# 583phoenix-hue/Airfoil-CFD-Tool

Measured on AMD Instinct MI355X. Metric: MLUPS on 4096² fp32 D2Q9 at 1/2/4/8 MI355X; achieved % HBM3E peak, higher is better.
Workload: dtype f32

## Files before the change

### airfoil-cfd-tool_amd/csrc/step_march3.hpp

```cpp
#pragma once
#include "step_march.hpp"

namespace wt {

static constexpr int M3_SREC = 80;
static constexpr int M3_SHALF = 40;
static constexpr int M3_HL = 32;
static constexpr int HL_COLS = 60;
static constexpr int H3_COLS = HL_COLS, H4_COLS = HL_COLS;


__global__ __launch_bounds__(256) void k_seam_flags3(const uint8_t *__restrict__ mask, const uint8_t *__restrict__ bcode, uint8_t *__restrict__ flags3,
                                                     Geom g, int nwin, int win)
{
    const long total = (long)(nwin - 1) * g.nxl;
    const long t = (long)blockIdx.x * 256 + threadIdx.x;
    if (t >= total) return;
    const int x = (int)(t % g.nxl);
    const int b = 1 + (int)(t / g.nxl);
    const uint8_t *m = mask + g.pitch;
    const int gi = x + g.gi0;
    unsigned f = 0;
    for (int r4 = 0; r4 < 4; r4++) {
        const int j = win * b - 2 + r4;
        if (j <= 0 || j >= g.ny - 1 || gi <= 0 || gi >= g.nx_g - 1) continue;
        const long c = (long)x * g.pitch + j;
        if (m[c] == 0 && bcode[c] == 0) f |= 1u << r4;
    }
    flags3[t] = (uint8_t)f;
}
__global__ __launch_bounds__(256) void k_seam_flags4(const uint8_t *__restrict__ mask, const uint8_t *__restrict__ bcode, uint8_t *__restrict__ flags4,
                                                     Geom g, int nwin, int win)
{
    const long total = (long)(nwin - 1) * g.nxl;
    const long t = (long)blockIdx.x * 256 + threadIdx.x;
    if (t >= total) return;
    const int x = (int)(t % g.nxl);
    const int b = 1 + (int)(t / g.nxl);
    const uint8_t *m = mask + g.pitch;
    const int gi = x + g.gi0;
    unsigned f = 0;
    for (int r6 = 0; r6 < 6; r6++) {
        const int j = win * b - 3 + r6;
        if (j <= 0 || j >= g.ny - 1 || gi <= 0 || gi >= g.nx_g - 1) continue;
        const long c = (long)x * g.pitch + j;
        if (m[c] == 0 && bcode[c] == 0) f |= 1u << r6;
    }
    flags4[t] = (uint8_t)f;
}

template <typename T, int FD, typename GET>
__device__ __forceinline__ void halo_step(unsigned sc, const Geom &g, int x, int j, bool plain, GET get, const FastDiv &fdv, T tau, T U0,
                                          T (&o)[9])
{
    if (j >= g.ny || x < 0 || x >= g.nxl) {
#pragma unroll
        for (int k = 0; k < 9; k++) o[k] = T(0);
        return;
    }
    const int gi = x + g.gi0;
    if (plain) {
        T fin[9], rho, ux, uy;
#pragma unroll
        for (int k = 0; k < 9; k++) fin[k] = get(k, -ex_of(k), -ey_of(k));
        collide_t<T, FD>(fin, fdv, tau, o, rho, ux, uy);
    } else if (sc & 256u) {
#pragma unroll
        for (int k = 0; k < 9; k++) o[k] = get(opp_of(k), 0, 0);
    } else if (gi == g.nx_g - 1) {
#pragma unroll
        for (int k = 0; k < 9; k++) o[k] = get(k, -1, 0);
    } else if (gi == 0 || j == g.ny - 1 || j == 0) {
        feq_all<T>(T(1), U0, T(0), o);
    } else {
        T fin[9], rho, ux, uy;
        fin[0] = get(0, 0, 0);
#pragma unroll
        for (int k = 1; k < 9; k++) fin[k] = ((sc >> (k - 1)) & 1u) ? get(opp_of(k), 0, 0) : get(k, -ex_of(k), -ey_of(k));
        collide_t<T, FD>(fin, fdv, tau, o, rho, ux, uy);
    }
}

#ifdef WT_UNIT_CLOCKS
__device__ unsigned long long g_halo_clk[8];
#define H4_STAMP(i) do { const unsigned long long t_ = __builtin_amdgcn_s_memtime(); hst_[i] = t_ - tprev_; tprev_ = t_; } while (0)
#else
#define H4_STAMP(i) do { } while (0)
#endif

template <typename T, int FD>
__device__ __forceinline__ void site_step1_seams(const T *__restrict__ rec, const T (&a)[9], int q0, unsigned sc, const Geom &g, int x, int j,
                                                 const FastDiv &fdv, T tau, T U0, T (&out)[9])
{
    const int gi = x + g.gi0;
    const int e0 = (q0 >> 2) * M3_SHALF + (q0 & 3);
    if (sc & 256u) {
#pragma unroll
        for (int k = 0; k < 9; k++) out[k] = rec[e0 + 4 * opp_of(k)];
    } else if (gi == g.nx_g - 1) {
#pragma unroll
        for (int k = 0; k < 9; k++) out[k] = rec[-M3_SREC + e0 + 4 * k];
    } else if (gi == 0 || j == g.ny - 1 || j == 0) {
        feq_all<T>(T(1), U0, T(0), out);
    } else {
        T fin[9], rho, ux, uy;
        fin[0] = a[0];
#pragma unroll
        for (int k = 1; k < 9; k++) fin[k] = ((sc >> (k - 1)) & 1u) ? rec[e0 + 4 * opp_of(k)] : a[k];
        collide_t<T, FD>(fin, fdv, tau, out, rho, ux, uy);
    }
}

template <typename T, int S, int FD, int DEPTH>
__device__ __forceinline__ void halo_lines_body(const T *__restrict__ fs, const T *__restrict__ seams3, const uint8_t *__restrict__ mask,
                                                const uint8_t *__restrict__ bcode, const uint8_t *__restrict__ flags, T *__restrict__ hl, const Geom &g, int nwin, int use_seams,
                                                const FastDiv &fdv, T tau, T U0, int xb0, int nbx)
{
    constexpr int WIN = 64 * S, NL = DEPTH - 1;
    constexpr int C1 = HL_COLS + 2 * NL, R1 = 2 * NL;
    constexpr int C2 = HL_COLS + 2 * (NL - 1), R2 = 2 * (NL - 1);
    constexpr int PADK = sizeof(T) == 4 ? 10 : 9;
    __shared__ __attribute__((aligned(32))) T l1[C1][R1][PADK];
    __shared__ T l2[DEPTH == 4 ? C2 : 1][DEPTH == 4 ? R2 : 1][9];
    __shared__ __attribute__((aligned(32))) T lv0[HL_COLS][2][4];
    static_assert(sizeof(T) * C1 * R1 * PADK >= sizeof(T) * HL_COLS * M3_HL, "the lines fit into l1");
    T (*ol)[M3_HL] = reinterpret_cast<T (*)[M3_HL]>(&l1[0][0][0]);
    const int b = 1 + (int)(blockIdx.x / nbx);
    const int x0 = (xb0 + (int)(blockIdx.x % nbx)) * HL_COLS;
    const uint8_t *m = mask + g.pitch;
    const T *s = fs + g.pitch;
    typedef T t4 __attribute__((ext_vector_type(4)));
#ifdef WT_UNIT_CLOCKS
    unsigned long long hst_[7] = {0, 0, 0, 0, 0, 0, 0}, tprev_ = __builtin_amdgcn_s_memtime();
#endif
    unsigned fl2 = 0, fl3 = 0, sc2 = 0, sc3 = 0;
    auto site_code = [&](int x, int j) -> unsigned {
        const long c = (long)x * g.pitch + j;
        return (unsigned)bcode[c] | (m[c] ? 256u : 0u);
    };
    if constexpr (DEPTH == 4) {
        const int x = x0 - (NL - 1) + (int)threadIdx.x / R2, j = WIN * b - (NL - 1) + (int)threadIdx.x % R2;
        if (x >= 0 && x < g.nxl) {
            fl2 = flags[(long)(b - 1) * g.nxl + x];
            if (j < g.ny && !((fl2 >> ((int)threadIdx.x % R2 + 1)) & 1)) sc2 = site_code(x, j);
        }
    }
    if (threadIdx.x < 2 * (HL_COLS + 2)) {
        const int x = x0 - 1 + (int)(threadIdx.x >> 1), j = WIN * b - 1 + (int)(threadIdx.x & 1);
        if (x >= 0 && x < g.nxl) {
            fl3 = flags[(long)(b - 1) * g.nxl + x];
            if (j < g.ny && !((fl3 >> (NL - 1 + (int)(threadIdx.x & 1))) & 1)) sc3 = site_code(x, j);
        }
    }
    for (int w = threadIdx.x; w < C1 * R1; w += 256) {
        const int cl = w / R1, r = w % R1;
        const int x = x0 - NL + cl;
        const int j = WIN * b - NL + r;
        T o[9];
#pragma unroll
        for (int k = 0; k < 9; k++) o[k] = T(0);
        if (x >= 0 && x < g.nxl && j < g.ny) {
            T a[9];
            const T *rec = seams3 + ((long)b * (g.nxl + 2) + x + 1) * M3_SREC;
#pragma unroll
            for (int k = 0; k < 9; k++) {
                const int q = 4 - NL + r - ey_of(k);
                a[k] = rec[-(long)ex_of(k) * M3_SREC + (q >> 2) * M3_SHALF + 4 * k + (q & 3)];
            }
            const bool plain = use_seams && ((flags[(long)(b - 1) * g.nxl + x] >> r) & 1) != 0;
            const int o0 = cl - NL;
            if ((r == NL || r == NL - 1) && o0 >= 0 && o0 < HL_COLS) {
                const bool below = r == NL;
                T v0 = below ? a[2] : a[4], v1 = below ? a[5] : a[7], v2 = below ? a[6] : a[8];
                if (!use_seams) {
                    const long c = (long)x * g.pitch + j;
                    if (below) { v0 = s[2 * g.plane + c - 1]; v1 = s[5 * g.plane + c - g.pitch - 1]; v2 = s[6 * g.plane + c + g.pitch - 1]; }
                    else { v0 = s[4 * g.plane + c + 1]; v1 = s[7 * g.plane + c + g.pitch + 1]; v2 = s[8 * g.plane + c - g.pitch + 1]; }
                }
                *reinterpret_cast<t4 *>(&lv0[o0][below ? 0 : 1][0]) = t4{v0, v1, v2, T(0)};
            }
            if (plain) {
                T rho, ux, uy;
                collide_t<T, FD>(a, fdv, tau, o, rho, ux, uy);
            } else if (use_seams) {
                site_step1_seams<T, FD>(rec, a, 4 - NL + r, site_code(x, j), g, x, j, fdv, tau, U0, o);
            } else {
                site_step1<T, FD>(s, m, g, x, j, fdv, tau, U0, o);
            }
        } else {
            const int o0 = cl - NL;
            if ((r == NL || r == NL - 1) && o0 >= 0 && o0 < HL_COLS) *reinterpret_cast<t4 *>(&lv0[o0][r == NL ? 0 : 1][0]) = t4{T(0), T(0), T(0), T(0)};
        }
#pragma unroll
        for (int k = 0; k < 9; k++) l1[cl][r][k] = o[k];
    }
    H4_STAMP(0);
    __syncthreads();
    H4_STAMP(1);
    if constexpr (DEPTH == 4) {
        static_assert(DEPTH != 4 || C2 * R2 == 256, "one level-2 item per thread");
        for (int w = threadIdx.x; w < C2 * R2; w += 256) {
            const int c2 = w / R2, r = w % R2;
            const int x = x0 - (NL - 1) + c2;
            const int j = WIN * b - (NL - 1) + r;
            const bool plain = ((fl2 >> (r + 1)) & 1) != 0;
            auto get = [&](int k, int dx, int dy) { return l1[c2 + 1 + dx][r + 1 + dy][k]; };
            T o[9];
            halo_step<T, FD>(sc2, g, x, j, plain, get, fdv, tau, U0, o);
#pragma unroll
            for (int k = 0; k < 9; k++) l2[c2][r][k] = o[k];
        }
        H4_STAMP(2);
        __syncthreads();
        H4_STAMP(3);
    }
    T wl[3] = {T(0), T(0), T(0)};
    t4 wq[3];
    const bool last_thr = threadIdx.x < 2 * (HL_COLS + 2), asm_thr = threadIdx.x >= 128 && threadIdx.x < 128 + 2 * HL_COLS;
    if (last_thr) {
        const int c = threadIdx.x >> 1, side = threadIdx.x & 1;
        const int x = x0 - 1 + c;
        const int j = WIN * b - 1 + side;
        const bool plain = ((fl3 >> (NL - 1 + side)) & 1) != 0;
        T o[9];
        if constexpr (DEPTH == 4) {
            auto get = [&](int k, int dx, int dy) { return l2[c + 1 + dx][1 + side + dy][k]; };
            halo_step<T, FD>(sc3, g, x, j, plain, get, fdv, tau, U0, o);
        } else {
            auto get = [&](int k, int dx, int dy) { return l1[c + 1 + dx][1 + side + dy][k]; };
            halo_step<T, FD>(sc3, g, x, j, plain, get, fdv, tau, U0, o);
        }
        wl[0] = side ? o[4] : o[2]; wl[1] = side ? o[8] : o[5]; wl[2] = side ? o[7] : o[6];
    } else if (asm_thr) {
        const int t = threadIdx.x - 128, o = t >> 1, side = t & 1;
        auto words = [&](const auto &lk, int c, int r) {
            return side == 0 ? t4{lk[c][r][2], lk[c - 1][r][5], lk[c + 1][r][6], T(0)} : t4{lk[c][r][4], lk[c + 1][r][7], lk[c - 1][r][8], T(0)};
        };
        wq[0] = words(l1, o + NL, NL - 1 + side);
        if constexpr (DEPTH == 4) wq[1] = words(l2, o + NL - 1, NL - 2 + side);
        wq[2] = *reinterpret_cast<const t4 *>(&lv0[o][side][0]);
    }
    H4_STAMP(4);
    __syncthreads();
    if (last_thr) {
        const int c = threadIdx.x >> 1, side = threadIdx.x & 1;
        const int base = 16 * side + 4 * (NL - 1);
        if (c >= 1 && c <= HL_COLS) { ol[c - 1][base] = wl[0]; ol[c - 1][base + 3] = T(0); }
        if (c < HL_COLS) ol[c][base + (side ? 2 : 1)] = wl[1];
        if (c >= 2) ol[c - 2][base + (side ? 1 : 2)] = wl[2];
    } else if (asm_thr) {
        const int t = threadIdx.x - 128, o = t >> 1, side = t & 1;
        *reinterpret_cast<t4 *>(&ol[o][16 * side]) = wq[0];
        if constexpr (DEPTH == 4) *reinterpret_cast<t4 *>(&ol[o][16 * side + 4]) = wq[1];
        *reinterpret_cast<t4 *>(&ol[o][16 * side + 12]) = wq[2];
    }
    __syncthreads();
    {
        const int nlines = g.nxl - x0 < HL_COLS ? g.nxl - x0 : HL_COLS;
        t4 *dst = reinterpret_cast<t4 *>(hl + ((long)b * (g.nxl + 2) + x0 + 1) * M3_HL);
        const t4 *src = reinterpret_cast<const t4 *>(&ol[0][0]);
        for (int t = threadIdx.x; t < nlines * (M3_HL / 4); t += 256) dst[t] = src[t];
    }
    H4_STAMP(5);
#ifdef WT_UNIT_CLOCKS
    if (threadIdx.x == 0) {
        for (int i = 0; i < 7; i++) atomicAdd(&g_halo_clk[i], hst_[i]);
        atomicAdd(&g_halo_clk[7], 1ULL);
    }
#endif
}

template <typename T, int S, int FD>
__global__ __launch_bounds__(256) void k_halo3(const T *__restrict__ fs, const T *__restrict__ seams3, const uint8_t *__restrict__ mask,
                                               const uint8_t *__restrict__ bcode, const uint8_t *__restrict__ flags3, T *__restrict__ hl, Geom g, int nwin, int use_seams,
                                               FastDiv fdv, T tau, T U0, int xb0, int nbx)
{
    halo_lines_body<T, S, FD, 3>(fs, seams3, mask, bcode, flags3, hl, g, nwin, use_seams, fdv, tau, U0, xb0, nbx);
}
template <typename T, int S, int FD>
__global__ __launch_bounds__(256) void k_halo4(const T *__restrict__ fs, const T *__restrict__ seams3, const uint8_t *__restrict__ mask,
                                               const uint8_t *__restrict__ bcode, const uint8_t *__restrict__ flags4, T *__restrict__ hl, Geom g, int nwin, int use_seams,
                                               FastDiv fdv, T tau, T U0, int xb0, int nbx)
{
    halo_lines_body<T, S, FD, 4>(fs, seams3, mask, bcode, flags4, hl, g, nwin, use_seams, fdv, tau, U0, xb0, nbx);
}


#ifdef WT_M3_STAMPS
__device__ unsigned long long g_m3_stamps[8];
#define M3_STAMP(i) do { const unsigned long long t_ = __builtin_amdgcn_s_memtime(); st_[i] += t_ - tprev_; tprev_ = t_; } while (0)
#else
#define M3_STAMP(i) do { } while (0)
#endif

template <typename T, int S>
struct March3Addr {
    MarchAddr<T, S> a;
    __amdgpu_buffer_rsrc_t rs3;
    unsigned voff_lo, voff_hi;
    T *lds_w;
    const char *lds_r;
};

template <bool BODY, bool WANT_MACRO, int FD, int LB, typename T, int S>
__device__ __forceinline__ void march_stage(const MarchParams<T> &p, int c, int j0, int lane, bool far_win, bool nf, bool allsolid,
                                            const T (&feq0)[9], const MV<T, S> (&m158)[3], const MV<T, S> (&Gc)[9], const MV<T, S> (&Gn)[9], T hv,
                                            MV<T, S> (&out)[9], MV<T, S> (&mac)[3], const uint32_t *pre = nullptr)
{
    typedef MV<T, S> V3;
    const Geom &g = p.g;
    constexpr bool OVL = (FD & MARCH_FD_OVL) != 0;
    V3 fin[9];
    fin[0] = Gc[0]; fin[1] = m158[0]; fin[3] = Gn[3];
    fin[2] = m_below_x<LB, OVL>(Gc[2], hv); fin[5] = m_below_x<LB + 1, OVL>(m158[1], hv); fin[6] = m_below_x<LB + 2, OVL>(Gn[6], hv);
    fin[4] = m_above_x<LB, OVL>(Gc[4], hv); fin[8] = m_above_x<LB + 2, OVL>(m158[2], hv); fin[7] = m_above_x<LB + 1, OVL>(Gn[7], hv);
    if (BODY) {
        const int gi = c + g.gi0;
        if (__builtin_expect(gi <= 0 || nf, 0)) {
            auto ownc = [&](int k) { return Gc[k]; };
            uint32_t solid4 = 0, code4 = 0;
            if (nf) {
                if (pre) { solid4 = pre[0]; code4 = pre[1]; }
                else {
                    solid4 = load_site_bytes<S>(p.mask + (long)(c + 1) * g.pitch + site_row<S, OVL>(j0, g.ny));
                    code4 = load_site_bytes<S>(p.bcode + (long)c * g.pitch + site_row<S, OVL>(j0, g.ny));
                }
            }
            const bool any_solid = __ballot(solid4 != 0) != 0ULL;
            if (gi <= 0) {
#pragma unroll
                for (int k = 0; k < 9; k++) out[k] = mv_splat<T, S>(feq0[k]);
                if (WANT_MACRO) { mac[0] = mv_splat<T, S>(T(1)); mac[1] = mv_splat<T, S>(p.U0); mac[2] = mv_splat<T, S>(T(0)); }
            } else if (allsolid) {
#pragma unroll
                for (int k = 0; k < 9; k++) out[k] = Gc[k];
                if (WANT_MACRO) { mac[0] = mv_splat<T, S>(T(1)); mac[1] = mv_splat<T, S>(T(0)); mac[2] = mv_splat<T, S>(T(0)); }
            } else {
                march_bounce<T, S>(fin, code4, ownc);
                march_collide_general<T, S, FD, WANT_MACRO>(fin, solid4, j0, g.ny, p.fdv, p.tau, p.U0, feq0, out, mac);
            }
            if (any_solid && (gi <= 0 || allsolid)) march_solid<T, S, WANT_MACRO>(out, mac, solid4, ownc);
            return;
        }
    }
    march_collide<T, S, FD, WANT_MACRO>(fin, p.fdv, p.tau, out, mac);
    if (far_win) march_far_rows<T, S, WANT_MACRO>(j0, g.ny, p.U0, feq0, out, mac);
}

template <bool EMIT, bool OVL = false, typename T, int S>
__device__ __forceinline__ void march3_store(const March3Addr<T, S> &m, unsigned voff_st, int col, const MV<T, S> (&out)[9], const MV<T, S> (&mac)[3])
{
    const MarchAddr<T, S> &a = m.a;
#pragma unroll
    for (int k = 0; k < 9; k++) bstore<T, S>(a.rd, voff_st, lat_off(a, k, col, 0), out[k]);
    if (EMIT) {
        const unsigned mo = (unsigned)col * a.pitch4;
#pragma unroll
        for (int q = 0; q < 3; q++) bstore<T, S>(a.rm, voff_st, (unsigned)q * a.mp4 + mo, mac[q]);
    }
    if constexpr (!OVL) {
#pragma unroll
        for (int k = 0; k < 9; k++) {
            u2v x;
            __builtin_memcpy(&x, &out[k], 8);
            *reinterpret_cast<u2v *>(m.lds_w + 4 * k) = x;
        }
    }
}
template <typename T, int S>
__device__ __forceinline__ void wait_for_column(const MV<T, S> (&c)[9], T h1)
{
#ifdef WT_M3_NOWAIT
    return;
#endif
    u2v r[9];
#pragma unroll
    for (int k = 0; k < 9; k++) __builtin_memcpy(&r[k], &c[k], 8);
    asm volatile("" ::"v"(r[0]), "v"(r[1]), "v"(r[2]), "v"(r[3]), "v"(r[4]), "v"(r[5]), "v"(r[6]), "v"(r[7]), "v"(r[8]), "v"(h1));
}
template <typename T, int S>
__device__ __forceinline__ void wait_for_column(const MV<T, S> (&c)[9], T h1, T h2)
{
    wait_for_column(c, h1);
#ifndef WT_M3_NOWAIT
    asm volatile("" ::"v"(h2));
#endif
}
template <typename T, int S>
__device__ __forceinline__ void wait_for_column(const MV<T, S> (&c)[9], T h1, T h2, T h3)
{
    wait_for_column(c, h1);
#ifndef WT_M3_NOWAIT
    asm volatile("" ::"v"(h2), "v"(h3));
#endif
}
__device__ __forceinline__ void wait_for_bytes(const SiteBytes &b)
{
#ifndef WT_M3_NOWAIT
    asm volatile("" ::"v"(b.v[0]), "v"(b.v[1]));
#endif
}
template <typename T, int S>
__device__ __forceinline__ void pin_after(const MV<T, S> (&c)[9])
{
    u2v r[9];
#pragma unroll
    for (int k = 0; k < 9; k++) __builtin_memcpy(&r[k], &c[k], 8);
    asm volatile("" ::"v"(r[0]), "v"(r[1]), "v"(r[2]), "v"(r[3]), "v"(r[4]), "v"(r[5]), "v"(r[6]), "v"(r[7]), "v"(r[8]));
}
struct Seam3 { u4v below, above; };
template <bool OVL = false, typename T, int S>
__device__ __forceinline__ Seam3 seam3_fetch(const March3Addr<T, S> &m)
{
    Seam3 r;
    if constexpr (OVL) { r.below = u4v{0, 0, 0, 0}; r.above = r.below; return r; }
    r.below = *reinterpret_cast<const u4v *>(m.lds_r);
    r.above = *reinterpret_cast<const u4v *>(m.lds_r + M3_SHALF * sizeof(T));
    return r;
}
template <bool OVL = false, typename T, int S>
__device__ __forceinline__ void seam3_flush(const March3Addr<T, S> &m, int col, const Seam3 &r)
{
    if constexpr (OVL) return;
    const unsigned so = (unsigned)(col + 1) * (unsigned)(M3_SREC * sizeof(T));
    const u4v d0 = r.below, d1 = r.above;
    __builtin_amdgcn_raw_buffer_store_b128(d0, m.rs3, m.voff_hi, so, 0);
    __builtin_amdgcn_raw_buffer_store_b128(d1, m.rs3, m.voff_lo, so, 0);
    store_data_fence2(d0, d1);
}

template <bool BODY, bool EMIT, int FD, typename T, int S>
__device__ __forceinline__ void march_unit3(const MarchParams<T> &p, March3Addr<T, S> &m, __amdgpu_buffer_rsrc_t rh, unsigned hoff,
                                            int ia, int ib, int uflags, int j0, int lane, bool far_win, ClassMask nonfast_m,
                                            ClassMask solid_m, const T (&feq0)[9])
{
    constexpr bool OVLF = (FD & MARCH_FD_OVL) != 0;
    typedef MV<T, S> V3;
    constexpr unsigned HREC = M3_HL * sizeof(T);
    const Geom &g = p.g;
    const MarchAddr<T, S> &a = m.a;
#define NONFAST(x) (BODY && cm_bit(nonfast_m, (x) - ia + 2))
#define ALLSOLID(x) (BODY && cm_bit(solid_m, (x) - ia + 2))
#define OWN_BUF(x) (a.own_lds + ((x) & 1) * OWN_LDS_BYTES)
#define OWN_NOW(x) do { if (BODY && NONFAST(x)) own_prefetch<T, S, OVLF>(a, (x), OWN_BUF(x)); } while (0)
#define STEP1(x, in, G) march_step1<BODY, FD, T, S, BODY>(p, a, (x), j0, far_win, NONFAST(x), ALLSOLID(x), feq0, in, G, nullptr, OWN_BUF(x))
#define STEP1P(x, in, G, sb) march_step1<BODY, FD, T, S, BODY>(p, a, (x), j0, far_win, NONFAST(x), ALLSOLID(x), feq0, in, G, BODY ? (sb).v : nullptr, OWN_BUF(x))
    const bool outlet = BODY && (uflags & MU_OUTLET_AFTER) != 0;
    const int xend = outlet ? ib : ib + 1;
    V3 s1m[3], s1c[9];
    V3 s2m[3], s2c[9];
    V3 in[9], G1[9], G2[9], mac[3];
#pragma unroll
    for (int k = 0; k < 9; k++) { s1c[k] = mv_splat<T, S>(feq0[k]); s2c[k] = s1c[k]; }
    s1m[0] = s1c[1]; s1m[1] = s1c[5]; s1m[2] = s1c[8];
    s2m[0] = s1c[1]; s2m[1] = s1c[5]; s2m[2] = s1c[8];
    T hv2 = halo_load_x<OVLF, T>(rh, hoff, (unsigned)(ia - 2 > 0 ? ia - 2 : 0) * HREC);
    T hv1 = halo_load_x<OVLF, T>(rh, hoff, (unsigned)(ia - 1 > 0 ? ia - 1 : 0) * HREC);
    T hv0 = halo_load_x<OVLF, T>(rh, hoff, (unsigned)ia * HREC);
    if (!BODY || ia - 2 + g.gi0 >= 0) {
        OWN_NOW(ia - 2);
        march_load_aligned(a, ia - 2, in);
        march_align_in<OVLF>(in, lane, hv2);
        STEP1(ia - 2, in, s1c);
    }
    s1m[0] = s1c[1]; s1m[1] = s1c[5]; s1m[2] = s1c[8];
    if (!BODY || ia - 1 + g.gi0 >= 0) {
        OWN_NOW(ia - 1);
        march_load_aligned(a, ia - 1, in);
        march_align_in<OVLF>(in, lane, hv1);
        STEP1(ia - 1, in, s1c);
    }
    OWN_NOW(ia);
    march_load_aligned(a, ia, in);
    SiteBytes sb0{{0, 0}}, sb1{{0, 0}}, sb2{{0, 0}};
    if (BODY) { sb0 = site_bytes_load<T, S, OVLF>(p, ia, j0); sb1 = site_bytes_load<T, S, OVLF>(p, ia - 1, j0); sb2 = site_bytes_load<T, S, OVLF>(p, ia - 2, j0); wait_for_bytes(sb0); wait_for_bytes(sb1); wait_for_bytes(sb2); }
    wait_for_column(in, hv0, hv1, hv2);
    int seam_col = -1;
#ifdef WT_M3_STAMPS
    unsigned long long st_[8] = {0, 0, 0, 0, 0, 0, 0, 0}, tprev_ = __builtin_amdgcn_s_memtime();
#endif
#pragma unroll 1
    for (int x = ia; x <= xend; x++) {
        V3 nxt[9];
        if (BODY && x + 1 <= xend && NONFAST(x + 1)) own_prefetch<T, S, OVLF>(a, x + 1, OWN_BUF(x + 1));
        march_load_aligned(a, (x + 1 <= xend) ? x + 1 : x, nxt);
        const bool has2 = x - 2 >= ia;
        const int c1 = x - 1, c2 = x - 2;
        const T hvn = halo_load_x<OVLF, T>(rh, hoff, (unsigned)(x + 1) * HREC);
        SiteBytes sbn{{0, 0}};
        if (BODY) sbn = site_bytes_load<T, S, OVLF>(p, x + 1, j0);
        const Seam3 sp = seam3_fetch<OVLF>(m);
        M3_STAMP(0);
        march_align_in<OVLF>(in, lane, hv0);
        STEP1P(x, in, G1, sb0);
        M3_STAMP(1);
        march_stage<BODY, false, FD, 0>(p, c1, j0, lane, far_win, NONFAST(c1), ALLSOLID(c1), feq0, s1m, s1c, G1, hv1, G2, mac, BODY ? sb1.v : nullptr);
#ifdef WT_M3_STAMPS
        pin_after(G2);
#endif
        M3_STAMP(2);
        V3 out[9];
        march_stage<BODY, EMIT, FD, 4>(p, c2, j0, lane, far_win, NONFAST(c2), ALLSOLID(c2), feq0, s2m, s2c, G2, hv2, out, mac, BODY ? sb2.v : nullptr);
        pin_after(out);
        M3_STAMP(3);
        wait_for_column(nxt, hvn);
        if (BODY) { wait_for_bytes(sbn); sb2 = sb1; sb1 = sb0; sb0 = sbn; }
#ifdef WT_M3_STAMPS
        asm volatile("s_waitcnt vmcnt(0)" ::: "memory");
#endif
        M3_STAMP(4);
        hv2 = hv1; hv1 = hv0; hv0 = hvn;
        march3_store<EMIT, OVLF>(m, has2 ? a.voff_st : p.lat_bytes, has2 ? c2 : 0, out, mac);
        seam3_flush<OVLF>(m, seam_col, sp);
        M3_STAMP(5);
        seam_col = has2 ? c2 : seam_col;
        if (BODY && outlet && x == xend) break;
        s2m[0] = s2c[1]; s2m[1] = s2c[5]; s2m[2] = s2c[8];
        s1m[0] = s1c[1]; s1m[1] = s1c[5]; s1m[2] = s1c[8];
#pragma unroll
        for (int k = 0; k < 9; k++) { s2c[k] = G2[k]; s1c[k] = G1[k]; in[k] = nxt[k]; }
    }
#ifdef WT_M3_STAMPS
    if (!BODY && lane == 0) {
        for (int i = 0; i < 6; i++) atomicAdd(&g_m3_stamps[i], st_[i]);
        atomicAdd(&g_m3_stamps[6], (unsigned long long)(xend - ia + 1));
        atomicAdd(&g_m3_stamps[7], 1ULL);
    }
#endif
    if (BODY && outlet) {
        const int co = ib;
        uint32_t solid4 = 0;
        if (NONFAST(co)) solid4 = load_site_bytes<S>(p.mask + (long)(co + 1) * g.pitch + site_row<S, OVLF>(j0, g.ny));
        const bool any_solid = __ballot(solid4 != 0) != 0ULL;
        V3 L2o[9], out[9];
#pragma unroll
        for (int k = 0; k < 9; k++) L2o[k] = s1c[k];
        if (any_solid) { auto own1 = [&](int k) { return G1[k]; }; march_solid<T, S, false>(L2o, mac, solid4, own1); }
        V3 t2m[3];
        t2m[0] = s2c[1]; t2m[1] = s2c[5]; t2m[2] = s2c[8];
        const T hv2t = halo_load_x<OVLF, T>(rh, hoff, (unsigned)(co - 1) * HREC);
        Seam3 sp = seam3_fetch<OVLF>(m);
        march_stage<BODY, EMIT, FD, 4>(p, co - 1, j0, lane, far_win, NONFAST(co - 1), ALLSOLID(co - 1), feq0, t2m, G2, L2o, hv2t, out, mac);
        march3_store<EMIT, OVLF>(m, a.voff_st, co - 1, out, mac);
        seam3_flush<OVLF>(m, seam_col, sp);
        seam_col = co - 1;
#pragma unroll
        for (int k = 0; k < 9; k++) out[k] = G2[k];
        if (EMIT) march_outlet_macro(G2, mac);
        if (any_solid) { auto own2 = [&](int k) { return L2o[k]; }; march_solid<T, S, EMIT>(out, mac, solid4, own2); }
        sp = seam3_fetch<OVLF>(m);
        march3_store<EMIT, OVLF>(m, a.voff_st, co, out, mac);
        seam3_flush<OVLF>(m, seam_col, sp);
        seam_col = co;
    }
    seam3_flush<OVLF>(m, seam_col, seam3_fetch<OVLF>(m));
#undef NONFAST
#undef ALLSOLID
#undef STEP1
#undef STEP1P
#undef OWN_BUF
#undef OWN_NOW
}

template <bool BODY, bool EMIT, int FD, typename T, int S>
__device__ __forceinline__ void march_unit4(const MarchParams<T> &p, March3Addr<T, S> &m, __amdgpu_buffer_rsrc_t rh,
                                            unsigned hoff, int ia, int ib, int uflags, int j0, int lane, bool far_win,
                                            ClassMask nonfast_m, ClassMask solid_m, const T (&feq0)[9])
{
    constexpr bool OVLF = (FD & MARCH_FD_OVL) != 0;
    typedef MV<T, S> V3;
    constexpr unsigned HREC = M3_HL * sizeof(T);
    const Geom &g = p.g;
    const MarchAddr<T, S> &a = m.a;
#define NONFAST(x) (BODY && (x) >= ia - 3 && cm_bit(nonfast_m, (x) - ia + 3))
#define ALLSOLID(x) (BODY && (x) >= ia - 3 && cm_bit(solid_m, (x) - ia + 3))
#define OWN_BUF(x) (a.own_lds + ((x) & 1) * OWN_LDS_BYTES)
#define OWN_NOW(x) do { if (BODY && NONFAST(x)) own_prefetch<T, S, OVLF>(a, (x), OWN_BUF(x)); } while (0)
#define STEP1(x, in, G) march_step1<BODY, FD, T, S, BODY>(p, a, (x), j0, far_win, NONFAST(x), ALLSOLID(x), feq0, in, G, nullptr, OWN_BUF(x))
#define HCOL(c) ((unsigned)((c) > 0 ? (c) : 0) * HREC)
    const bool outlet = BODY && (uflags & MU_OUTLET_AFTER) != 0;
    const int xend = outlet ? ib : ib + 2;
    V3 s1m[3], s1c[9];
    V3 s2m[3], s2c[9];
    V3 s3m[3], s3c[9];
    V3 in[9], G1[9], G2[9], G3[9], mac[3];
#pragma unroll
    for (int k = 0; k < 9; k++) { s1c[k] = mv_splat<T, S>(feq0[k]); s2c[k] = s1c[k]; s3c[k] = s1c[k]; }
    s1m[0] = s1c[1]; s1m[1] = s1c[5]; s1m[2] = s1c[8];
    s2m[0] = s1c[1]; s2m[1] = s1c[5]; s2m[2] = s1c[8];
    s3m[0] = s1c[1]; s3m[1] = s1c[5]; s3m[2] = s1c[8];
    const int xs = ia - 1;
#define LCOL(x) ((BODY && (x) + g.gi0 < 0) ? -g.gi0 : (x))
    T hv3 = halo_load_x<OVLF, T>(rh, hoff, HCOL(xs - 3)), hv2 = halo_load_x<OVLF, T>(rh, hoff, HCOL(xs - 2)), hv1 = halo_load_x<OVLF, T>(rh, hoff, HCOL(xs - 1)),
      hv0 = halo_load_x<OVLF, T>(rh, hoff, HCOL(xs));
    if (!BODY || ia - 3 + g.gi0 >= 0) {
        OWN_NOW(ia - 3);
        march_load_aligned(a, ia - 3, in);
        march_align_in<OVLF>(in, lane, hv2);
        STEP1(ia - 3, in, s1c);
    }
    s1m[0] = s1c[1]; s1m[1] = s1c[5]; s1m[2] = s1c[8];
    if (!BODY || ia - 2 + g.gi0 >= 0) {
        OWN_NOW(ia - 2);
        march_load_aligned(a, ia - 2, in);
        march_align_in<OVLF>(in, lane, hv1);
        STEP1(ia - 2, in, s1c);
    }
    OWN_NOW(xs);
    march_load_aligned(a, LCOL(xs), in);
    SiteBytes sb0{{0, 0}}, sb1{{0, 0}}, sb2{{0, 0}}, sb3{{0, 0}};
    if (BODY) {
        sb0 = site_bytes_load<T, S, OVLF>(p, xs, j0); sb1 = site_bytes_load<T, S, OVLF>(p, xs - 1, j0); sb2 = site_bytes_load<T, S, OVLF>(p, xs - 2, j0); sb3 = site_bytes_load<T, S, OVLF>(p, xs - 3, j0);
        wait_for_bytes(sb0); wait_for_bytes(sb1); wait_for_bytes(sb2); wait_for_bytes(sb3);
    }
    wait_for_column(in, hv0, hv1, hv2);
    wait_for_column(in, hv3);
    int seam_col = -1;
#pragma unroll 1
    for (int x = xs; x <= xend; x++) {
        V3 nxt[9];
        if (BODY && x + 1 <= xend && NONFAST(x + 1)) own_prefetch<T, S, OVLF>(a, x + 1, OWN_BUF(x + 1));
        march_load_aligned(a, (x + 1 <= xend) ? x + 1 : x, nxt);
        const bool has3 = x - 3 >= ia;
        const int c1 = x - 1, c2 = x - 2, c3 = x - 3;
        const T hvn = halo_load_x<OVLF, T>(rh, hoff, HCOL(x + 1));
        SiteBytes sbn{{0, 0}};
        if (BODY) sbn = site_bytes_load<T, S, OVLF>(p, x + 1, j0);
        const Seam3 sp = seam3_fetch<OVLF>(m);
        march_align_in<OVLF>(in, lane, hv0);
        march_step1<BODY, FD, T, S, BODY>(p, a, x, j0, far_win, NONFAST(x), ALLSOLID(x), feq0, in, G1, BODY ? sb0.v : nullptr, OWN_BUF(x));

        march_stage<BODY, false, FD, 0>(p, c1, j0, lane, far_win, NONFAST(c1), ALLSOLID(c1), feq0, s1m, s1c, G1, hv1, G2, mac, BODY ? sb1.v : nullptr);
        march_stage<BODY, false, FD, 4>(p, c2, j0, lane, far_win, NONFAST(c2), ALLSOLID(c2), feq0, s2m, s2c, G2, hv2, G3, mac, BODY ? sb2.v : nullptr);
        V3 out[9];
        march_stage<BODY, EMIT, FD, 8>(p, c3, j0, lane, far_win, NONFAST(c3), ALLSOLID(c3), feq0, s3m, s3c, G3, hv3, out, mac, BODY ? sb3.v : nullptr);
        pin_after(out);
        wait_for_column(nxt, hvn);
        if (BODY) { wait_for_bytes(sbn); sb3 = sb2; sb2 = sb1; sb1 = sb0; sb0 = sbn; }
        hv3 = hv2; hv2 = hv1; hv1 = hv0; hv0 = hvn;
        march3_store<EMIT, OVLF>(m, has3 ? a.voff_st : p.lat_bytes, has3 ? c3 : 0, out, mac);
        seam3_flush<OVLF>(m, seam_col, sp);
        seam_col = has3 ? c3 : seam_col;
        if (BODY && outlet && x == xend) break;
        s3m[0] = s3c[1]; s3m[1] = s3c[5]; s3m[2] = s3c[8];
        s2m[0] = s2c[1]; s2m[1] = s2c[5]; s2m[2] = s2c[8];
        s1m[0] = s1c[1]; s1m[1] = s1c[5]; s1m[2] = s1c[8];
#pragma unroll
        for (int k = 0; k < 9; k++) { s3c[k] = G3[k]; s2c[k] = G2[k]; s1c[k] = G1[k]; in[k] = nxt[k]; }
    }
    if (BODY && outlet) {
        const int co = ib;
        uint32_t solid4 = 0;
        if (NONFAST(co)) solid4 = load_site_bytes<S>(p.mask + (long)(co + 1) * g.pitch + site_row<S, OVLF>(j0, g.ny));
        const bool any_solid = __ballot(solid4 != 0) != 0ULL;
        V3 O2[9], O3[9], L3a[9], out[9], tm[3];
#pragma unroll
        for (int k = 0; k < 9; k++) O2[k] = s1c[k];
        if (any_solid) { auto own = [&](int k) { return G1[k]; }; march_solid<T, S, false>(O2, mac, solid4, own); }
        tm[0] = s2c[1]; tm[1] = s2c[5]; tm[2] = s2c[8];
        march_stage<BODY, false, FD, 4>(p, co - 1, j0, lane, far_win, NONFAST(co - 1), ALLSOLID(co - 1), feq0, tm, G2, O2, halo_load_x<OVLF, T>(rh, hoff, HCOL(co - 1)), L3a, mac);
#pragma unroll
        for (int k = 0; k < 9; k++) O3[k] = G2[k];
        if (any_solid) { auto own = [&](int k) { return O2[k]; }; march_solid<T, S, false>(O3, mac, solid4, own); }
        tm[0] = s3c[1]; tm[1] = s3c[5]; tm[2] = s3c[8];
        Seam3 sp = seam3_fetch<OVLF>(m);
        const bool own2 = co - 2 >= ia;
        march_stage<BODY, EMIT, FD, 8>(p, co - 2, j0, lane, far_win, NONFAST(co - 2), ALLSOLID(co - 2), feq0, tm, G3, L3a, halo_load_x<OVLF, T>(rh, hoff, HCOL(co - 2)), out, mac);
        march3_store<EMIT, OVLF>(m, own2 ? a.voff_st : p.lat_bytes, own2 ? co - 2 : 0, out, mac);
        seam3_flush<OVLF>(m, seam_col, sp);
        seam_col = own2 ? co - 2 : seam_col;
        tm[0] = G3[1]; tm[1] = G3[5]; tm[2] = G3[8];
        sp = seam3_fetch<OVLF>(m);
        march_stage<BODY, EMIT, FD, 8>(p, co - 1, j0, lane, far_win, NONFAST(co - 1), ALLSOLID(co - 1), feq0, tm, L3a, O3, halo_load_x<OVLF, T>(rh, hoff, HCOL(co - 1)), out, mac);
        march3_store<EMIT, OVLF>(m, a.voff_st, co - 1, out, mac);
        seam3_flush<OVLF>(m, seam_col, sp);
        seam_col = co - 1;
#pragma unroll
        for (int k = 0; k < 9; k++) out[k] = L3a[k];
        if (EMIT) march_outlet_macro(L3a, mac);
        if (any_solid) { auto own = [&](int k) { return O3[k]; }; march_solid<T, S, EMIT>(out, mac, solid4, own); }
        sp = seam3_fetch<OVLF>(m);
        march3_store<EMIT, OVLF>(m, a.voff_st, co, out, mac);
        seam3_flush<OVLF>(m, seam_col, sp);
        seam_col = co;
    }
    seam3_flush<OVLF>(m, seam_col, seam3_fetch<OVLF>(m));
#undef NONFAST
#undef ALLSOLID
#undef STEP1
#undef OWN_BUF
#undef OWN_NOW
#undef HCOL
#undef LCOL
}

template <bool BODY, bool EMIT, int FD, typename T, int S>
__device__ __forceinline__ void march_unit3_d2(const MarchParams<T> &p, March3Addr<T, S> &m, __amdgpu_buffer_rsrc_t rh, unsigned hoff, int ia, int ib,
                                               int uflags, int j0, int lane, bool far_win, ClassMask nonfast_m, ClassMask solid_m,
                                               const T (&feq0)[9])
{
    constexpr bool OVLF = (FD & MARCH_FD_OVL) != 0;
    typedef MV<T, S> V3;
    constexpr unsigned HREC = M3_HL * sizeof(T);
    const Geom &g = p.g;
    const MarchAddr<T, S> &a = m.a;
#define NONFAST(x) (BODY && cm_bit(nonfast_m, (x) - ia + 2))
#define ALLSOLID(x) (BODY && cm_bit(solid_m, (x) - ia + 2))
#define STEP1(x, in, G) march_step1<BODY, FD, T, S>(p, a, (x), j0, far_win, NONFAST(x), ALLSOLID(x), feq0, in, G)
    const bool outlet = BODY && (uflags & MU_OUTLET_AFTER) != 0;
    const int xend = ib;
    V3 s1m[3], s1c[9];
    V3 in[9], G1[9], mac[3];
#pragma unroll
    for (int k = 0; k < 9; k++) s1c[k] = mv_splat<T, S>(feq0[k]);
    s1m[0] = s1c[1]; s1m[1] = s1c[5]; s1m[2] = s1c[8];
    T hv1 = halo_load_x<OVLF, T>(rh, hoff, (unsigned)(ia - 1 > 0 ? ia - 1 : 0) * HREC), hv0 = halo_load_x<OVLF, T>(rh, hoff, (unsigned)ia * HREC);
    if (!BODY || ia - 1 + g.gi0 >= 0) {
        march_load_aligned(a, ia - 1, in);
        march_align_in<OVLF>(in, lane, hv1);
        STEP1(ia - 1, in, s1c);
    }
    march_load_aligned(a, ia, in);
    wait_for_column(in, hv0, hv1);
    int seam_col = -1;
#pragma unroll 1
    for (int x = ia; x <= xend; x++) {
        V3 nxt[9];
        march_load_aligned(a, (x + 1 <= xend) ? x + 1 : x, nxt);
        const bool has1 = x - 1 >= ia;
        const int c1 = x - 1;
        const T hvn = halo_load_x<OVLF, T>(rh, hoff, (unsigned)(x + 1) * HREC);
        const Seam3 sp = seam3_fetch<OVLF>(m);
        march_align_in<OVLF>(in, lane, hv0);
        STEP1(x, in, G1);
        V3 out[9];
        march_stage<BODY, EMIT, FD, 0>(p, c1, j0, lane, far_win, NONFAST(c1), ALLSOLID(c1), feq0, s1m, s1c, G1, hv1, out, mac);
        pin_after(out);
        wait_for_column(nxt, hvn);
        hv1 = hv0; hv0 = hvn;
        march3_store<EMIT, OVLF>(m, has1 ? a.voff_st : p.lat_bytes, has1 ? c1 : 0, out, mac);
        seam3_flush<OVLF>(m, seam_col, sp);
        seam_col = has1 ? c1 : seam_col;
        if (BODY && outlet && x == xend) break;
        s1m[0] = s1c[1]; s1m[1] = s1c[5]; s1m[2] = s1c[8];
#pragma unroll
        for (int k = 0; k < 9; k++) { s1c[k] = G1[k]; in[k] = nxt[k]; }
    }
    if (BODY && outlet) {
        const int co = ib;
        uint32_t solid4 = 0;
        if (NONFAST(co)) solid4 = load_site_bytes<S>(p.mask + (long)(co + 1) * g.pitch + site_row<S, OVLF>(j0, g.ny));
        V3 out[9];
#pragma unroll
        for (int k = 0; k < 9; k++) out[k] = s1c[k];
        if (EMIT) march_outlet_macro(s1c, mac);
        if (__ballot(solid4 != 0) != 0ULL) { auto own1 = [&](int k) { return G1[k]; }; march_solid<T, S, EMIT>(out, mac, solid4, own1); }
        const Seam3 sp = seam3_fetch<OVLF>(m);
        march3_store<EMIT, OVLF>(m, a.voff_st, co, out, mac);
        seam3_flush<OVLF>(m, seam_col, sp);
        seam_col = co;
    }
    seam3_flush<OVLF>(m, seam_col, seam3_fetch<OVLF>(m));
#undef NONFAST
#undef ALLSOLID
#undef STEP1
}

static inline MarchRange march_range3(const Geom &g, int depth = 3)
{
    MarchRange r;
    r.i_begin = (g.gi0 == 0) ? 0 : depth - 1;
    r.outlet_after = (g.gi0 + g.nxl == g.nx_g) ? 1 : 0;
    r.i_end = r.outlet_after ? g.nxl - 1 : g.nxl - (depth - 1);
    return r;
}

}
```

Before: 225,500.

## Rewrite fp32 halo-line kernel to process site pairs per thread with packed collide

Adds a new fp32 halo-lines body in which each thread handles two vertically adjacent sites, uses packed f2v loads from LDS and a paired collide routine, and stages intermediate levels in padded LDS with odd-bank column strides. Plain fluid pairs take a fast path with no per-site boundary classification, and assembly of the output lines is split between two thread groups. The aim is to cut per-site overhead and LDS bank conflicts in the halo kernel. The cost is more complex code and more registers per thread. The fp64 path still uses the old body.

```diff
diff --git a/airfoil-cfd-tool_amd/csrc/step_march3.hpp b/airfoil-cfd-tool_amd/csrc/step_march3.hpp
--- a/airfoil-cfd-tool_amd/csrc/step_march3.hpp
+++ b/airfoil-cfd-tool_amd/csrc/step_march3.hpp
@@ -270,19 +270,309 @@
 #endif
 }
 
+struct HaloSite {
+    unsigned rev;
+    bool outlet;
+    bool far;
+    bool zero;
+    bool keep;
+};
+__device__ __forceinline__ HaloSite halo_site(unsigned sc, const Geom &g, int x, int j)
+{
+    HaloSite h;
+    const int gi = x + g.gi0;
+    h.zero = j >= g.ny || x < 0 || x >= g.nxl;
+    const bool solid = (sc & 256u) != 0;
+    h.outlet = !solid && gi == g.nx_g - 1;
+    h.far = !h.zero && !solid && !h.outlet && (gi == 0 || j == g.ny - 1 || j == 0);
+    h.rev = solid ? 0x1ffu : ((h.outlet || h.far) ? 0u : (sc & 0xffu) << 1);
+    h.keep = h.zero || solid || h.outlet || h.far;
+    return h;
+}
+template <int I, typename FETCH>
+__device__ __forceinline__ void halo_inputs(const HaloSite &h, const float (&fq)[9], FETCH fetch, f2v (&fin)[9])
+{
+#pragma unroll
+    for (int k = 0; k < 9; k++) {
+        const bool rev = ((h.rev >> k) & 1u) != 0;
+        const int kk = rev ? opp_of(k) : k;
+        const int dx = rev ? 0 : (h.outlet ? -1 : -ex_of(k));
+        const int dy = (rev || h.outlet) ? 0 : -ey_of(k);
+        float v = 0.0f;
+        if (!h.zero && !h.far) v = fetch(I, kk, dx, dy);
+        fin[k][I] = h.far ? fq[k] : v;
+    }
+}
+template <int FD>
+__device__ __forceinline__ void halo_collide_pair(const f2v (&fin)[9], const bool (&keep)[2], const FastDiv &fdv, f2v (&o)[9])
+{
+    if constexpr ((FD & MARCH_FD_CONTRACTED) != 0) {
+#pragma unroll
+        for (int i = 0; i < 2; i++) {
+            float a[9], f[9], r, u, w;
+#pragma unroll
+            for (int k = 0; k < 9; k++) a[k] = fin[k][i];
+            collide_contracted(a, fdv.rtau, f, r, u, w);
+#pragma unroll
+            for (int k = 0; k < 9; k++) o[k][i] = f[k];
+        }
+    } else {
+        f2v r, u, w;
+        collide2_packed<(FD & 3), (FD & MARCH_FD_TWOOP) != 0>(fin, fdv, o, r, u, w);
+    }
+#pragma unroll
+    for (int k = 0; k < 9; k++) {
+        o[k][0] = keep[0] ? fin[k][0] : o[k][0];
+        o[k][1] = keep[1] ? fin[k][1] : o[k][1];
+    }
+}
+__host__ __device__ constexpr int halo_col_stride(int R) { return (((9 * R) / 2) & 1) ? 9 * R : 9 * R + 2; }
+
+template <int R, int CS, int FD>
+__device__ __forceinline__ void halo_step_pair(const float *pe, bool pl0, bool pl1, const unsigned (&sc)[2], const Geom &g, int x, int j0, const FastDiv &fdv,
+                                               float U0, f2v (&o)[9])
+{
+    f2v fin[9];
+    bool keep[2] = {false, false};
+    if (pl0 && pl1) {
+#pragma unroll
+        for (int k = 0; k < 9; k++) {
+            const float *q = pe - ex_of(k) * CS + k * R + 1 - ey_of(k);
+            if (ey_of(k) != 0) fin[k] = *reinterpret_cast<const f2v *>(q);
+            else fin[k] = f2v{q[0], q[1]};
+        }
+    } else {
+        float fq[9];
+        feq_all<float>(1.0f, U0, 0.0f, fq);
+        auto fetch = [&](int i, int kk, int dx, int dy) { return pe[dx * CS + kk * R + 1 + i + dy]; };
+        const HaloSite h0 = halo_site(sc[0], g, x, j0), h1 = halo_site(sc[1], g, x, j0 + 1);
+        halo_inputs<0>(h0, fq, fetch, fin);
+        halo_inputs<1>(h1, fq, fetch, fin);
+        keep[0] = h0.keep; keep[1] = h1.keep;
+    }
+    halo_collide_pair<FD>(fin, keep, fdv, o);
+}
+
+template <int S, int FD, int DEPTH>
+__device__ __forceinline__ void halo_lines_body2(const float *__restrict__ fs, const float *__restrict__ seams3, const uint8_t *__restrict__ mask,
+                                                 const uint8_t *__restrict__ bcode, const uint8_t *__restrict__ flags, float *__restrict__ hl, const Geom &g, int nwin,
+                                                 int use_seams, const FastDiv &fdv, float U0, int xb0, int nbx)
+{
+    typedef float T;
+    constexpr int WIN = 64 * S, NL = DEPTH - 1;
+    constexpr int C1 = HL_COLS + 2 * NL, R1 = 2 * NL;
+    constexpr int C2 = HL_COLS + 2 * (NL - 1), R2 = 2 * (NL - 1);
+    constexpr int CL = HL_COLS + 2;
+    constexpr int CS1 = halo_col_stride(R1), CS2 = halo_col_stride(R2);
+    constexpr int N1 = C1 * NL, N2 = C2 * (R2 / 2);
+    static_assert(N1 <= 256 && N2 <= 128 && CL <= 128, "every level is one trip of the workgroup; the assembling threads are 128 .. 247");
+    __shared__ __attribute__((aligned(32))) T l1[C1 * CS1];
+    __shared__ __attribute__((aligned(32))) T l2[DEPTH == 4 ? C2 * CS2 : 2];
+    __shared__ __attribute__((aligned(32))) T lv0[HL_COLS][2][4];
+    static_assert(C1 * CS1 >= HL_COLS * M3_HL, "the lines fit into l1");
+    T (*ol)[M3_HL] = reinterpret_cast<T (*)[M3_HL]>(&l1[0]);
+    const int b = 1 + (int)(blockIdx.x / nbx);
+    const int x0 = (xb0 + (int)(blockIdx.x % nbx)) * HL_COLS;
+    const int tid = (int)threadIdx.x;
+    const uint8_t *m = mask + g.pitch;
+    const T *s = fs + g.pitch;
+    typedef T t4 __attribute__((ext_vector_type(4)));
+#ifdef WT_UNIT_CLOCKS
+    unsigned long long hst_[7] = {0, 0, 0, 0, 0, 0, 0}, tprev_ = __builtin_amdgcn_s_memtime();
+#endif
+    unsigned fl2 = 0, fl3 = 0, sc2[2] = {0, 0}, sc3[2] = {0, 0};
+    auto site_code = [&](int x, int j) -> unsigned {
+        const long c = (long)x * g.pitch + j;
+        return (unsigned)bcode[c] | (m[c] ? 256u : 0u);
+    };
+    if constexpr (DEPTH == 4) {
+        const int x = x0 - (NL - 1) + tid / (R2 / 2), r0 = 2 * (tid % (R2 / 2));
+        if (tid < N2 && x >= 0 && x < g.nxl) {
+            fl2 = flags[(long)(b - 1) * g.nxl + x];
+#pragma unroll
+            for (int i = 0; i < 2; i++) {
+                const int j = WIN * b - (NL - 1) + r0 + i;
+                if (j < g.ny && !((fl2 >> (r0 + i + 1)) & 1)) sc2[i] = site_code(x, j);
+            }
+        }
+    }
+    if (tid < CL) {
+        const int x = x0 - 1 + tid;
+        if (x >= 0 && x < g.nxl) {
+            fl3 = flags[(long)(b - 1) * g.nxl + x];
+#pragma unroll
+            for (int i = 0; i < 2; i++) {
+                const int j = WIN * b - 1 + i;
+                if (j < g.ny && !((fl3 >> (NL - 1 + i)) & 1)) sc3[i] = site_code(x, j);
+            }
+        }
+    }
+    if (tid < N1) {
+        const int cl = tid / NL, r0 = 2 * (tid % NL);
+        const int x = x0 - NL + cl, j0 = WIN * b - NL + r0;
+        const bool xin = x >= 0 && x < g.nxl;
+        const int o0 = cl - NL;
+        const bool line_col = o0 >= 0 && o0 < HL_COLS;
+        const T *rec = seams3 + ((long)b * (g.nxl + 2) + x + 1) * M3_SREC;
+        const long c0 = (long)x * g.pitch + j0;
+        f2v fin[9];
+#pragma unroll
+        for (int k = 0; k < 9; k++) fin[k] = f2v{0.0f, 0.0f};
+        bool keep[2] = {true, true};
+        bool inr[2];
+#pragma unroll
+        for (int i = 0; i < 2; i++) inr[i] = xin && j0 + i < g.ny;
+        auto fetch_rec = [&](int i, int kk, int dx, int dy) {
+            const int q = 4 - NL + r0 + i + dy;
+            return rec[(long)dx * M3_SREC + (q >> 2) * M3_SHALF + 4 * kk + (q & 3)];
+        };
+        auto fetch_lat = [&](int i, int kk, int dx, int dy) { return s[(long)kk * g.plane + c0 + i + (long)dx * g.pitch + dy]; };
+        if (use_seams) {
+            unsigned fl1 = 0;
+#pragma unroll
+            for (int i = 0; i < 2; i++) {
+                if (inr[i]) {
+#pragma unroll
+                    for (int k = 0; k < 9; k++) fin[k][i] = fetch_rec(i, k, -ex_of(k), -ey_of(k));
+                }
+            }
+            if (xin) fl1 = flags[(long)(b - 1) * g.nxl + x];
+#pragma unroll
+            for (int i = 0; i < 2; i++) {
+                const int r = r0 + i;
+                if ((r == NL || r == NL - 1) && line_col) {
+                    const bool below = r == NL;
+                    *reinterpret_cast<t4 *>(&lv0[o0][below ? 0 : 1][0]) =
+                        t4{below ? fin[2][i] : fin[4][i], below ? fin[5][i] : fin[7][i], below ? fin[6][i] : fin[8][i], T(0)};
+                }
+            }
+            const bool pl[2] = {((fl1 >> r0) & 1) != 0, ((fl1 >> (r0 + 1)) & 1) != 0};
+            keep[0] = keep[1] = false;
+            if (!(pl[0] && pl[1])) {
+                float fq[9];
+                feq_all<float>(1.0f, U0, 0.0f, fq);
+                if (!pl[0]) {
+                    const HaloSite h = halo_site(inr[0] ? site_code(x, j0) : 0u, g, x, j0);
+                    halo_inputs<0>(h, fq, fetch_rec, fin);
+                    keep[0] = h.keep;
+                }
+                if (!pl[1]) {
+                    const HaloSite h = halo_site(inr[1] ? site_code(x, j0 + 1) : 0u, g, x, j0 + 1);
+                    halo_inputs<1>(h, fq, fetch_rec, fin);
+                    keep[1] = h.keep;
+                }
+            }
+        } else {
+            float fq[9];
+            feq_all<float>(1.0f, U0, 0.0f, fq);
+            const HaloSite h0 = halo_site(inr[0] ? site_code(x, j0) : 0u, g, x, j0), h1 = halo_site(inr[1] ? site_code(x, j0 + 1) : 0u, g, x, j0 + 1);
+            halo_inputs<0>(h0, fq, fetch_lat, fin);
+            halo_inputs<1>(h1, fq, fetch_lat, fin);
+            keep[0] = h0.keep; keep[1] = h1.keep;
+#pragma unroll
+            for (int i = 0; i < 2; i++) {
+                const int r = r0 + i;
+                if ((r == NL || r == NL - 1) && line_col) {
+                    const bool below = r == NL;
+                    T v0 = T(0), v1 = T(0), v2 = T(0);
+                    if (inr[i]) {
+                        const long c = c0 + i;
+                        if (below) { v0 = s[2 * g.plane + c - 1]; v1 = s[5 * g.plane + c - g.pitch - 1]; v2 = s[6 * g.plane + c + g.pitch - 1]; }
+                        else { v0 = s[4 * g.plane + c + 1]; v1 = s[7 * g.plane + c + g.pitch + 1]; v2 = s[8 * g.plane + c - g.pitch + 1]; }
+                    }
+                    *reinterpret_cast<t4 *>(&lv0[o0][below ? 0 : 1][0]) = t4{v0, v1, v2, T(0)};
+                }
+            }
+        }
+        f2v o[9];
+        halo_collide_pair<FD>(fin, keep, fdv, o);
+#pragma unroll
+        for (int k = 0; k < 9; k++) *reinterpret_cast<f2v *>(&l1[cl * CS1 + k * R1 + r0]) = o[k];
+    }
+    H4_STAMP(0);
+    __syncthreads();
+    H4_STAMP(1);
+    if constexpr (DEPTH == 4) {
+        if (tid < N2) {
+            const int c2 = tid / (R2 / 2), r0 = 2 * (tid % (R2 / 2));
+            f2v o[9];
+            halo_step_pair<R1, CS1, FD>(&l1[(c2 + 1) * CS1 + r0], ((fl2 >> (r0 + 1)) & 1) != 0, ((fl2 >> (r0 + 2)) & 1) != 0, sc2, g, x0 - (NL - 1) + c2,
+                                        WIN * b - (NL - 1) + r0, fdv, U0, o);
+#pragma unroll
+            for (int k = 0; k < 9; k++) *reinterpret_cast<f2v *>(&l2[c2 * CS2 + k * R2 + r0]) = o[k];
+        }
+        H4_STAMP(2);
+        __syncthreads();
+        H4_STAMP(3);
+    }
+    T wl[2][3] = {{T(0), T(0), T(0)}, {T(0), T(0), T(0)}};
+    t4 wq[3];
+    const bool last_thr = tid < CL, asm_thr = tid >= 128 && tid < 128 + 2 * HL_COLS;
+    if (last_thr) {
+        f2v o[9];
+        const bool pl0 = ((fl3 >> (NL - 1)) & 1) != 0, pl1 = ((fl3 >> NL) & 1) != 0;
+        if constexpr (DEPTH == 4) halo_step_pair<R2, CS2, FD>(&l2[(tid + 1) * CS2], pl0, pl1, sc3, g, x0 - 1 + tid, WIN * b - 1, fdv, U0, o);
+        else halo_step_pair<R1, CS1, FD>(&l1[(tid + 1) * CS1], pl0, pl1, sc3, g, x0 - 1 + tid, WIN * b - 1, fdv, U0, o);
+        wl[0][0] = o[2][0]; wl[0][1] = o[5][0]; wl[0][2] = o[6][0];
+        wl[1][0] = o[4][1]; wl[1][1] = o[8][1]; wl[1][2] = o[7][1];
+    } else if (asm_thr) {
+        const int t = tid - 128, o = t >> 1, side = t & 1;
+        auto words = [&](const T *lk, int cs, int rr, int c, int r) {
+            const T *q = lk + c * cs + r;
+            return side == 0 ? t4{q[2 * rr], q[5 * rr - cs], q[6 * rr + cs], T(0)} : t4{q[4 * rr], q[7 * rr + cs], q[8 * rr - cs], T(0)};
+        };
+        wq[0] = words(l1, CS1, R1, o + NL, NL - 1 + side);
+        if constexpr (DEPTH == 4) wq[1] = words(l2, CS2, R2, o + NL - 1, NL - 2 + side);
+        wq[2] = *reinterpret_cast<const t4 *>(&lv0[o][side][0]);
+    }
+    H4_STAMP(4);
+    __syncthreads();
+    if (last_thr) {
+        const int c = tid;
+#pragma unroll
+        for (int side = 0; side < 2; side++) {
+            const int base = 16 * side + 4 * (NL - 1);
+            if (c >= 1 && c <= HL_COLS) { ol[c - 1][base] = wl[side][0]; ol[c - 1][base + 3] = T(0); }
+            if (c < HL_COLS) ol[c][base + (side ? 2 : 1)] = wl[side][1];
+            if (c >= 2) ol[c - 2][base + (side ? 1 : 2)] = wl[side][2];
+        }
+    } else if (asm_thr) {
+        const int t = tid - 128, o = t >> 1, side = t & 1;
+        *reinterpret_cast<t4 *>(&ol[o][16 * side]) = wq[0];
+        if constexpr (DEPTH == 4) *reinterpret_cast<t4 *>(&ol[o][16 * side + 4]) = wq[1];
+        *reinterpret_cast<t4 *>(&ol[o][16 * side + 12]) = wq[2];
+    }
+    __syncthreads();
+    {
+        const int nlines = g.nxl - x0 < HL_COLS ? g.nxl - x0 : HL_COLS;
+        t4 *dst = reinterpret_cast<t4 *>(hl + ((long)b * (g.nxl + 2) + x0 + 1) * M3_HL);
+        const t4 *src = reinterpret_cast<const t4 *>(&ol[0][0]);
+        for (int t = tid; t < nlines * (M3_HL / 4); t += 256) dst[t] = src[t];
+    }
+    H4_STAMP(5);
+#ifdef WT_UNIT_CLOCKS
+    if (tid == 0) {
+        for (int i = 0; i < 7; i++) atomicAdd(&g_halo_clk[i], hst_[i]);
+        atomicAdd(&g_halo_clk[7], 1ULL);
+    }
+#endif
+}
+
 template <typename T, int S, int FD>
 __global__ __launch_bounds__(256) void k_halo3(const T *__restrict__ fs, const T *__restrict__ seams3, const uint8_t *__restrict__ mask,
                                                const uint8_t *__restrict__ bcode, const uint8_t *__restrict__ flags3, T *__restrict__ hl, Geom g, int nwin, int use_seams,
                                                FastDiv fdv, T tau, T U0, int xb0, int nbx)
 {
-    halo_lines_body<T, S, FD, 3>(fs, seams3, mask, bcode, flags3, hl, g, nwin, use_seams, fdv, tau, U0, xb0, nbx);
+    if constexpr (sizeof(T) == 4) halo_lines_body2<S, FD, 3>(fs, seams3, mask, bcode, flags3, hl, g, nwin, use_seams, fdv, U0, xb0, nbx);
+    else halo_lines_body<T, S, FD, 3>(fs, seams3, mask, bcode, flags3, hl, g, nwin, use_seams, fdv, tau, U0, xb0, nbx);
 }
 template <typename T, int S, int FD>
 __global__ __launch_bounds__(256) void k_halo4(const T *__restrict__ fs, const T *__restrict__ seams3, const uint8_t *__restrict__ mask,
                                                const uint8_t *__restrict__ bcode, const uint8_t *__restrict__ flags4, T *__restrict__ hl, Geom g, int nwin, int use_seams,
                                                FastDiv fdv, T tau, T U0, int xb0, int nbx)
 {
-    halo_lines_body<T, S, FD, 4>(fs, seams3, mask, bcode, flags4, hl, g, nwin, use_seams, fdv, tau, U0, xb0, nbx);
+    if constexpr (sizeof(T) == 4) halo_lines_body2<S, FD, 4>(fs, seams3, mask, bcode, flags4, hl, g, nwin, use_seams, fdv, U0, xb0, nbx);
+    else halo_lines_body<T, S, FD, 4>(fs, seams3, mask, bcode, flags4, hl, g, nwin, use_seams, fdv, tau, U0, xb0, nbx);
 }
 
 
```

After: 219,400. 0.973x the previous value.
